# fverdoja/Fast-3D-Pointcloud-Segmentation

Hardware: AMD Instinct MI355X
Metric: Mpoints/sec segmented end-to-end, 1M-pt RGB-D frames (higher is better)
Workload: dtype f32

## Files before the change

__graft_entry__.py:

```python
import importlib
import os
import subprocess
import sys

ROOT = os.path.dirname(os.path.abspath(__file__))
PKG = "fast-3d-pointcloud-segmentation_amd"


def _run(cmd):
    print("+", " ".join(cmd), flush=True)
    subprocess.run(cmd, check=True)


def build() -> None:
    _run(["make", "-C", os.path.join(ROOT, PKG, "csrc")])
    _run(["make", "-C", os.path.join(ROOT, "oracle")])
    _run(["make", "-C", os.path.join(ROOT, "tests", "emul")])
    _run(["make", "-C", os.path.join(ROOT, "tests", "devprobe")])
    _run(["make", "-C", os.path.join(ROOT, "tests", "kernprobe")])
    _run(["make", "-C", os.path.join(ROOT, "tests", "blockprobe")])
    if ROOT not in sys.path:
        sys.path.insert(0, ROOT)
    P = importlib.import_module(PKG)
    lib = P.load_library()
    assert lib.f3ds_version() >= 120
    P.check_library_is_current(lib)


def smoke() -> None:
    import ctypes
    import numpy as np
    if ROOT not in sys.path:
        sys.path.insert(0, ROOT)
    sys.path.insert(0, os.path.join(ROOT, "tests"))
    P = importlib.import_module(PKG)
# ... 22 lines not shown
```

fast-3d-pointcloud-segmentation_amd/csrc/f3ds_hip.hip:

```cpp
#include <hip/hip_runtime.h>

#include <algorithm>
#include <cmath>
#include <atomic>
#include <map>
#include <chrono>
#include <cstdio>
#include <cstdlib>
#include <cstring>
#include <string>
#include <type_traits>
#include <mutex>
#include <set>
#include <vector>

#include "../../include/f3ds.h"
#include "f3ds_algo.h"
#include "f3ds_glasbey.h"
#include "f3ds_eval.h"
#include "f3ds_dev.h"
#include "f3ds_levels.h"
#include "f3ds_eval_levels.h"

using namespace f3ds;
// ... 45 lines not shown
template <class K>
hipError_t launch_fn(uint32_t gx, uint32_t nf, uint32_t lds, hipStream_t st, const void* dargs) {
    using Pack = pack_of<K>;
    if (lds > 48u * 1024u) {
        hipError_t e = hipFuncSetAttribute(reinterpret_cast<const void*>(k_batched<K, Pack>), hipFuncAttributeMaxDynamicSharedMemorySize, (int)lds);
        if (e != hipSuccess) return e;
    }
    hipLaunchKernelGGL((k_batched<K, Pack>), dim3(gx ? gx : 1u, nf), dim3(K::BLOCK), lds, st, static_cast<const Pack*>(dargs));
    return hipGetLastError();
}
struct Cmd { LaunchFn fn; uint32_t gx, lds, bytes, off; };

const int g_inc_shift = [] { const char* e = dev_getenv("F3DS_INC_SHIFT"); return e ? atoi(e) : 6; }();

struct Switches {
    bool direct_labels = false, copy_stream = true, copy_duplex = false, split_voxel_accum = false, sweep_tiles = true, merge_spec = true, force_global_merge = false, no_stream_pool = false, sort_pairs = false, host_prof = false, trace_err = false, vox_hash = true, vox_tiles_forced = false, levels_global = false;
    int normals_threads = 0, merge_nw = 0, merge_keys = -1; uint32_t tile_holes = 0, ilist_slack = 32, r_rounds = F3DS_R_ROUNDS, grid_cap = 0; long relabel_lds_cap = -1;
    void read() {
        auto on = [](const char* n) { return dev_getenv(n) != nullptr; };
        auto num = [](const char* n, long dflt) { const char* e = dev_getenv(n); return e ? atol(e) : dflt; };
        direct_labels = num("F3DS_DIRECT_LABELS", 0) != 0; copy_stream = num("F3DS_COPY_STREAM", 1) != 0; copy_duplex = num("F3DS_COPY_STREAM", 1) == 2; split_voxel_accum = on("F3DS_SPLIT_VOXEL_ACCUM"); sweep_tiles = num("F3DS_SWEEP_TILES", 1) != 0; merge_spec = num("F3DS_MERGE_SPEC", 1) != 0;
        force_global_merge = on("F3DS_FORCE_GLOBAL_MERGE"); no_stream_pool = on("F3DS_NO_STREAM_POOL"); sort_pairs = on("F3DS_SORT_PAIRS");
        host_prof = on("F3DS_HOST_PROF"); trace_err = on("F3DS_TRACE_ERR");
        vox_tiles_forced = num("F3DS_VOX_TILES", 1) == 2;
        vox_hash = num("F3DS_VOX_TILES", 1) != 0 && !sort_pairs && !split_voxel_accum;
        normals_threads = (int)num("F3DS_NORMALS_THREADS", 0); tile_holes = (uint32_t)num("F3DS_SWEEP_TILE_HOLES", 0);
        { const long v = num("F3DS_MERGE_NW", 0); merge_nw = v == 4 ? 4 : (v ? 8 : 0); }
        { const char* e = dev_getenv("F3DS_MERGE_KEYS"); merge_keys = !e ? -1 : (!strcmp(e, "lds") ? 2 : (!strcmp(e, "global") ? 1 : 0)); }
        relabel_lds_cap = num("F3DS_RELABEL_LDS_CAP", -1);
        levels_global = num("F3DS_LEVELS_GLOBAL", 0) != 0;
        { const long v = num("F3DS_R_ROUNDS_RUN", F3DS_R_ROUNDS); r_rounds = v >= 1 && v <= F3DS_R_ROUNDS ? (uint32_t)v : (uint32_t)F3DS_R_ROUNDS; }
        { const long v = num("F3DS_ILIST_SLACK", 32); ilist_slack = v >= 1 && v <= 32 ? (uint32_t)v : 32u; }
        { const long v = num("F3DS_GRID_CAP", 0); grid_cap = v >= 1 && v <= 2048 ? (uint32_t)v : 0u; }
    }
};
thread_local Switches g_sw;
const int g_merge_shared_res = [] { const char* e = dev_getenv("F3DS_MERGE_SHARED_RES"); return e && atoi(e) == 2 ? 2 : 0; }();

#define F3DS_SCRATCH(X) \
    X(P16, pts) X(P16, spts) X(uint64_t, keys0) X(uint64_t, keys1) X(uint32_t, vals0) X(uint32_t, vals1) X(uint32_t, flags) X(uint32_t, incl) X(uint32_t, tiles) X(uint32_t, hist) X(uint32_t, seg_start) X(int, pt_voxel) X(uint32_t, labels) \
// ... 283 lines not shown
    HIPCHECK(timed_sync(b.st));
    HIPCHECK(hipGetLastError());
    if (nf > 1) for (size_t i = 0; i < nf; ++i) *b.fr[i]->h_dc = b.owner->h_dcblk[i];
    return F3DS_OK;
}

int scan_u32(f3ds_ctx* c, const uint32_t* in, uint32_t* out, uint32_t n) {
    const uint32_t nt = n ? (n + SCAN_TILE - 1) / SCAN_TILE : 1u;
    uint32_t* tiles;
    ENSURE(c->tiles, nt, tiles);
    rec<d_scan_tiles>(c, nt, 0u, in, out, tiles, n);
    rec<d_scan_single>(c, 1u, 0u, tiles, nt);
    rec<d_scan_add>(c, nt, 0u, out, tiles, n);
    return F3DS_OK;
}
int radix_sort(f3ds_ctx* c, uint64_t* k0, uint32_t* v0, uint64_t* k1, uint32_t* v1, uint32_t n, int total_bits, uint64_t** keys_out, uint32_t** vals_out, int base_shift = 0, const uint32_t* n_dev = nullptr) {
    *keys_out = k0; if (vals_out) *vals_out = v0;
    if (total_bits <= 0) return F3DS_OK;
    const int passes = (total_bits + RS_MAXBITS - 1) / RS_MAXBITS;
    const int per = (total_bits + passes - 1) / passes;
    const uint32_t nb = n ? (n + RS_TILE - 1) / RS_TILE : 1u;
    uint32_t* hist;
    ENSURE(c->hist, (size_t)RS_BINS * nb, hist);
    int shift = 0;
    for (int p = 0; p < passes; ++p) {
        const int bits = (total_bits - shift) < per ? (total_bits - shift) : per;
        rec<d_radix_hist>(c, nb, 0u, k0, n, base_shift + shift, bits, hist, nb, n_dev);
        rec<d_scan_single>(c, 1u, 0u, hist, (uint32_t)((1u << bits) * nb));
        if (v0) rec<d_radix_scatter>(c, nb, 0u, k0, v0, k1, v1, n, base_shift + shift, bits, hist, nb, n_dev);
        else rec<d_radix_scatter_k>(c, nb, 0u, k0, k1, n, base_shift + shift, bits, hist, nb);
        std::swap(k0, k1); std::swap(v0, v1);
        shift += bits;
    }
    *keys_out = k0; if (vals_out) *vals_out = v0;
    return F3DS_OK;
}

int seg_bbox(f3ds_ctx* c) {
    rec<d_init_counters>(c, 1u, 0u, c->d_dc);
    rec<d_bbox>(c, grid_for(c->n, 256 * 8) < 512 ? grid_for(c->n, 256 * 8) : 512u, 0u, c->d_pts, c->n, c->fa, c->d_dc);
    rec<d_grid>(c, 1u, 0u, c->d_dc, c->prm.voxel_res, c->d_grid);
    return F3DS_OK;
}
int seg_sort(f3ds_ctx* c, int sort_bits, int idxbits) {
// ... 15 lines not shown
        if ((rc = scan_u32(c, flags, incl, n))) return rc;
        rec<d_segstart>(c, grid_for(n, 256), 0u, c->ks, flags, incl, n, invalid, seg_start, &c->d_dc->n_voxels, &c->d_dc->n_valid, ks);
        return F3DS_OK;
    }
    const uint32_t nt = n ? (n + SCAN_TILE - 1) / SCAN_TILE : 1u;
    uint32_t* tiles; ENSURE(c->tiles, nt, tiles);
    rec<d_seg_count>(c, nt, 0u, c->ks, n, invalid, ks, tiles);
    rec<d_scan_single>(c, 1u, 0u, tiles, nt);
    rec<d_seg_write>(c, nt, 0u, c->ks, n, invalid, ks, tiles, seg_start, &c->d_dc->n_voxels, &c->d_dc->n_valid);
    return F3DS_OK;
}
int seg_vox_tiles(f3ds_ctx* c, int code_bits, int tile_bits) {
    const uint32_t n = c->n;
    const uint32_t ntiles = (n + VT_TILE - 1u) / VT_TILE;
    const uint64_t dcap64 = (uint64_t)ntiles * VT_ENT_MAX;
    if (code_bits + tile_bits + VT_CNT_BITS > 64 || dcap64 > 0x7fffffffull || (uint64_t)ntiles * VT_TAB > 0x7fffffffull) return F3DS_ERR_UNSUPPORTED;
    const uint32_t dcap = (uint32_t)dcap64;
    const uint64_t fin = c->h_dc->n_finite;
    const uint32_t capV = (uint32_t)std::max<uint64_t>(256u, std::min<uint64_t>(fin, dcap));
    c->vox_cap = capV;
    uint64_t *k0, *k1; uint32_t *ploc, *v0, *v1, *part, *vkey, *vcount, *seg_start, *list; uint2* bo_te; float* vf; int* pt_voxel;
    const uint32_t nchunks = (dcap + DS_CHUNK - 1u) / DS_CHUNK;
    ENSURE(c->pslot, n, ploc); ENSURE(c->keys0, dcap, k0); ENSURE(c->keys1, dcap, k1); ENSURE(c->vals0, dcap, v0); ENSURE(c->vals1, dcap, v1);
    { uint32_t* w; ENSURE(c->hcnt, (size_t)ntiles * VT_TAB * 2 + 2u * nchunks, w); bo_te = reinterpret_cast<uint2*>(w); part = w + (size_t)ntiles * VT_TAB * 2; }
    ENSURE(c->vkey, (size_t)capV * 3, vkey); ENSURE(c->vcount, capV, vcount); ENSURE(c->vf, (size_t)capV * 12, vf);
    ENSURE(c->seg_start, (size_t)capV + 1, seg_start); ENSURE(c->vlist, n, list); ENSURE(c->pt_voxel, n, pt_voxel);
    { uint32_t *f, *incl; ENSURE(c->flags, capV, f); ENSURE(c->incl, capV, incl); }
    c->idxbits = -1; c->ks = nullptr; c->vs = nullptr;
    rec<d_tile_keys>(c, std::min<uint32_t>(ntiles, (uint32_t)g_grid_cap * 16u), 0u, c->d_pts, n, c->fa, c->d_grid, ploc, k0, v0, dcap, tile_bits, c->d_dc);
    uint64_t* ks; uint32_t* vs;
    int rc = radix_sort(c, k0, v0, k1, v1, dcap, code_bits + tile_bits, &ks, &vs, VT_CNT_BITS, &c->d_dc->seg_count);
    if (rc) return rc;
    rec<d_desc_part>(c, nchunks, 0u, ks, dcap, tile_bits, part, c->d_dc);
    rec<d_desc_offsets>(c, 1u, 0u, part, dcap, capV, seg_start, c->d_dc);
    rec<d_desc_apply>(c, nchunks, 0u, ks, vs, dcap, capV, tile_bits, c->fa, c->d_grid, part, bo_te, seg_start, vkey, c->d_dc);
    rec<d_tile_place>(c, std::min<uint32_t>(ntiles, (uint32_t)g_grid_cap * 16u), 0u, ploc, n, bo_te, list, pt_voxel, c->d_dc);
    rec<d_voxel_list_accum>(c, std::min<uint32_t>(grid_wide(capV, 256), std::max<uint32_t>(64u, grid_wide(n / 8u, 256))), 0u, c->d_pts, list, seg_start, c->fa, vf, vcount, c->d_dc, capV);
    c->vox_hashed = true;
    return F3DS_OK;
}
int seg_neighbors(f3ds_ctx* c, uint32_t wgs) {
    const uint32_t V = c->V;
    const bool blocks = c->h_dc->depth <= N_BLOCK_DEPTH_MAX;
    const uint32_t cap = blocks ? pow2_ge((size_t)V + 16) : pow2_ge((size_t)V * 2 + 16);
    const size_t words = blocks ? (size_t)cap * 2 : cap;
    uint32_t* hvals = nullptr; int *nbr, *nbrT; uint64_t* hkeys;
    c->hmask = cap - 1;
    ENSURE(c->nbr, (size_t)V * 27, nbr); ENSURE(c->nbrT, (size_t)V * 27, nbrT); ENSURE(c->hkeys, words, hkeys);
    if (!blocks) ENSURE(c->hvals, cap, hvals);
    rec_fill(c, hkeys, 0xFFFFFFFFu, words * 8);
    rec<d_vox_table>(c, wgs, 0u, c->vkey.p, V, c->d_grid, hkeys, hvals, c->hmask);
// ... 559 lines not shown
    bool hashed = g_sw.vox_hash && (nctx >= 4 || g_sw.vox_tiles_forced);
    for (f3ds_ctx* c : b.fr) {
        c->vox_hashed = false;
        if (c->vox_dense && hashed) { if (c->vox_dense_wait) c->vox_dense_wait--; else c->vox_dense = false; }
    }
    for (f3ds_ctx* c : b.fr) if (c->vox_dense) hashed = false;
    if (hashed) {
        uint32_t maxtiles = 1;
        for (f3ds_ctx* c : b.fr) maxtiles = std::max(maxtiles, (c->n + VT_TILE - 1u) / VT_TILE);
        const int tile_bits = bits_for((uint64_t)maxtiles - 1u);
        rc = for_frames(b, [&](f3ds_ctx* c) { return seg_vox_tiles(c, 3 * maxd, tile_bits); });
        if (rc == F3DS_ERR_UNSUPPORTED) {
            for (f3ds_ctx* c : b.fr) { reset_recording(c); c->vox_hashed = false; }
            hashed = false;
        } else if (rc || (rc = flush_sync(b))) return rc;
        if (hashed && g_sw.trace_err) for (f3ds_ctx* c : b.fr) fprintf(stderr, "f3ds: tile path: most voxels in a tile %u, descriptors %u, leaves %u, lists sorted %u\n", c->h_dc->vox_max_tile, c->h_dc->seg_count, c->h_dc->n_voxels, c->h_dc->vox_disorder);
        if (hashed) for (f3ds_ctx* c : b.fr) if (c->h_dc->ev_overflow == 6 || c->h_dc->ev_overflow == 7) {
            if (g_sw.trace_err) fprintf(stderr, "f3ds: tile path refused a frame: %s (descriptors %u, leaves %u)\n", c->h_dc->ev_overflow == 6 ? "a voxel with too many points" : "a tile with too many voxels", c->h_dc->seg_count, c->h_dc->n_voxels);
            c->vox_dense = true; c->vox_dense_wait = c->vox_dense_penalty; c->vox_dense_penalty = std::min(2u * c->vox_dense_penalty, 1024u); hashed = false;
        }
        if (!hashed) {
            if (g_sw.trace_err) fprintf(stderr, "f3ds: voxelisation of %zu frames runs again on the sort path (an unorganised cloud or dense voxels)\n", b.fr.size());
            for (f3ds_ctx* c : b.fr) {
                c->vox_hashed = false;
                if ((rc = clear_counters(c, b.st, &DevCounters::error, &DevCounters::ev_overflow, &DevCounters::n_voxels, &DevCounters::seg_count))) return rc;
            }
        }
    }
    if (!hashed) {
        uint32_t maxn = 1;
        for (f3ds_ctx* c : b.fr) if (c->n > maxn) maxn = c->n;
// ... 944 lines not shown
```

fast-3d-pointcloud-segmentation_amd/csrc/f3ds_kernels.inc:

```


namespace {

struct P16 { float x, y, z; uint32_t rgba; };

struct DevCounters {
    unsigned long long n_finite;
    uint32_t bbox[6];
    uint32_t bbox_any;
    uint32_t n_valid;
    uint32_t n_voxels;
    uint32_t n_cells;
    uint32_t n_seeds;
    uint32_t n_edges;
    uint32_t n_alive;
    uint32_t n_merges;
    uint32_t n_regions;
    uint32_t n_events;
    int error;
    int r_overflow;
    float lambda;
    uint32_t seg_count;
    uint32_t n_ghosts;
    int depth;
// ... 251 lines not shown
            uint64_t peers = __ballot(valid);
            for (int b = 0; b < bits; ++b) {
                uint64_t m = __ballot(valid && ((d >> b) & 1u));
                peers &= ((d >> b) & 1u) ? m : ~m;
            }
            uint32_t pos = 0;
            if (valid) pos = wcount[w][d] + (uint32_t)__popcll(peers & lanemask_lt());
            __builtin_amdgcn_wave_barrier();
            if (valid && (peers & lanemask_lt()) == 0ull) wcount[w][d] += (uint32_t)__popcll(peers);
            __builtin_amdgcn_wave_barrier();
            if (valid) keys_out[pos] = k[s];
        }
    }
};

struct FrameArgs {
    int use_transform, fold_negative_z, leaf_order;
    float voxel_res, seed_res, w_color, w_spatial, w_normal;
};

__device__ inline P16 load_point(const P16* pts, size_t i) {
    const uint4 q = reinterpret_cast<const uint4*>(pts)[i];
    P16 p;
    p.x = __uint_as_float(q.x); p.y = __uint_as_float(q.y); p.z = __uint_as_float(q.z); p.rgba = q.w;
    return p;
}

__device__ inline bool vt_blocks(int depth) { return depth <= N_BLOCK_DEPTH_MAX; }
constexpr uint32_t BT_EMPTY = 0xFFFFFFFFu;
struct __attribute__((aligned(16))) BtEntry { uint32_t key, base; unsigned long long vacant; };
// ... 283 lines not shown
            vcount[v] = cnt;
            uint64_t code = keys[s] >> keyshift;
            if (fa.leaf_order == 1) code = (~code) & ((1ull << (3 * depth)) - 1ull);
            unsigned k[3];
            n_demorton(code, depth, k);
            vkey[v * 3] = k[0]; vkey[v * 3 + 1] = k[1]; vkey[v * 3 + 2] = k[2];
        }
    }
};

#ifndef F3DS_VT_TILE
#define F3DS_VT_TILE 4096
#endif
constexpr uint32_t VT_TILE = F3DS_VT_TILE;
constexpr uint32_t VT_TAB = VT_TILE / 2;
constexpr int VT_CNT_BITS = 14;
static_assert(VT_TILE < (1u << VT_CNT_BITS), "a tile's point count must fit the count field");
constexpr uint32_t VT_ENT_MAX = VT_TAB * 5 / 8;
constexpr uint32_t VL_MAX_RUN = 256;
constexpr uint32_t VOX_NONE = 0xFFFFFFFFu;
__device__ inline void run_of_lane(bool valid, uint32_t w0, uint32_t w1, bool* head, int* head_lane, uint32_t* run_len) {
    const int lane = lane_id();
    const uint32_t p0 = __shfl_up(w0, 1, 64), p1 = __shfl_up(w1, 1, 64);
    const bool pv = __shfl_up((int)valid, 1, 64) != 0;
    const bool h = valid && (lane == 0 || !pv || p0 != w0 || p1 != w1);
    const uint64_t hm = __ballot(h), vm = __ballot(valid);
    const uint64_t le = lane == 63 ? ~0ull : ((2ull << lane) - 1ull);
    const int hl = valid ? 63 - __builtin_clzll(hm & le) : lane;
    const uint64_t above = hl == 63 ? 0ull : ~((2ull << hl) - 1ull);
    const uint64_t stop = (hm | ~vm) & above;
    *head = h; *head_lane = hl; *run_len = (uint32_t)((stop ? __builtin_ctzll(stop) : 64) - hl);
}
struct d_tile_keys {
    static constexpr int BLOCK = 256;
    __device__ void operator()(const P16* pts, uint32_t n, FrameArgs fa, const GridInfo* gp, uint32_t* ploc, uint64_t* dkeys, uint32_t* dvals,
                               uint32_t dcap, int tile_bits, DevCounters* dc) const {
        __shared__ unsigned long long tkey[VT_TAB];
        __shared__ uint32_t tcnt[VT_TAB];
        __shared__ uint32_t tbits[2][VT_TAB / 32];
        __shared__ uint32_t s_ent, s_base, s_over[2], s_dis;
        const GridInfo g = *gp;
        const uint64_t code_mask = (1ull << (3 * g.depth)) - 1ull;
        const int lane = lane_id();
        const uint32_t tid = threadIdx.x;
        const uint32_t ntiles = (n + VT_TILE - 1u) / VT_TILE;
        for (uint32_t tile = BIX; tile < ntiles; tile += gridDim.x) {
            for (uint32_t e = tid; e < VT_TAB; e += 256u) { tkey[e] = HASH_EMPTY; tcnt[e] = 0u; }
            if (tid < VT_TAB / 32u) { tbits[0][tid] = 0u; tbits[1][tid] = 0u; }
            if (tid == 0) { s_ent = 0u; s_over[0] = 0u; s_over[1] = 0u; s_dis = 0u; }
            __syncthreads();
            const uint32_t t0 = tile * VT_TILE, t1 = n - t0 < VT_TILE ? n : t0 + VT_TILE;
            constexpr uint32_t VT_PF = 4;
            uint32_t it4 = 0u;
            for (uint32_t base4 = t0; base4 < t1 && !s_over[(it4 + 1u) & 1u]; base4 += 256u * VT_PF, ++it4) {
              uint4 q[VT_PF];
        #pragma unroll
              for (uint32_t j = 0; j < VT_PF; ++j) { const uint32_t i = base4 + j * 256u + tid; q[j] = reinterpret_cast<const uint4*>(pts)[i < t1 ? i : t1 - 1u]; }
        #pragma unroll
              for (uint32_t j = 0; j < VT_PF; ++j) {
                const uint32_t base = base4 + j * 256u;
                if (base >= t1) break;
                const uint32_t i = base + tid;
                const uint32_t step = (base - t0) >> 8;
                uint64_t pk = HASH_EMPTY;
                if (i < t1) {
                    float x = __uint_as_float(q[j].x), y = __uint_as_float(q[j].y), z = __uint_as_float(q[j].z);
                    n_prelude(z, fa.fold_negative_z);
                    if (n_finite3(x, y, z) && !g.empty) { unsigned k[3]; n_point_key(g, x, y, z, fa.use_transform, k); pk = n_pack_key(k[0], k[1], k[2]); }
                }
// ... 5 lines not shown
                    uint32_t e = (uint32_t)hash64(pk) & (VT_TAB - 1u);
                    for (uint32_t probes = 0; probes < VT_TAB; ++probes) {
                        const unsigned long long old = atomicCAS(&tkey[e], (unsigned long long)HASH_EMPTY, (unsigned long long)pk);
                        if (old == HASH_EMPTY) { if (atomicAdd(&s_ent, 1u) >= VT_ENT_MAX) s_over[it4 & 1u] = 1u; ent = e; break; }
                        if (old == pk) { ent = e; break; }
                        e = (e + 1u) & (VT_TAB - 1u);
                    }
                    if (ent != VOX_NONE) {
                        roff = atomicAdd(&tcnt[ent], len);
                        const uint32_t bit = 1u << (ent & 31u);
                        if (atomicOr(&tbits[step & 1u][ent >> 5], bit) & bit) s_dis = 1u;
                    } else s_over[it4 & 1u] = 1u;
                }
                if (tid < VT_TAB / 32u) tbits[(step + 1u) & 1u][tid] = 0u;
                ent = __shfl(ent, hl, 64); roff = __shfl(roff, hl, 64);
                if (i < t1) ploc[i] = (valid && ent != VOX_NONE) ? (ent << 16) | (roff + (uint32_t)(lane - hl)) : VOX_NONE;
                __syncthreads();
              }
            }
            __syncthreads();
            if (tid == 0) { atomicMax(&dc->vox_max_tile, s_ent); if (s_dis) dc->vox_disorder = 1u; }
            if (s_over[0] | s_over[1]) { if (tid == 0) { dc->error = F3DS_ERR_UNSUPPORTED; dc->ev_overflow = 7; } return; }
            if (tid == 0) s_base = s_ent ? atomicAdd(&dc->seg_count, s_ent) : 0u;
            __syncthreads();
            const uint32_t dbase = s_base;
            if (tid == 0) s_ent = 0u;
            __syncthreads();
            for (uint32_t e0 = 0; e0 < VT_TAB; e0 += 256u) {
                const uint32_t e = e0 + tid;
                const unsigned long long pk = tkey[e];
                const bool live = pk != HASH_EMPTY;
                const uint64_t lm = __ballot(live);
                if (!lm) continue;
                uint32_t wb = 0;
                if (lane == __builtin_ctzll(lm)) wb = atomicAdd(&s_ent, (uint32_t)__popcll(lm));
                wb = __shfl(wb, __builtin_ctzll(lm), 64);
                if (live) {
                    const uint32_t d = dbase + wb + (uint32_t)__popcll(lm & lanemask_lt());
                    if (d < dcap) {
                        uint64_t code = n_morton((unsigned)(pk >> 42) & 0x1FFFFFu, (unsigned)(pk >> 21) & 0x1FFFFFu, (unsigned)pk & 0x1FFFFFu, g.depth);
                        if (fa.leaf_order == 1) code = (~code) & code_mask;
                        dkeys[d] = (((code << tile_bits) | (uint64_t)tile) << VT_CNT_BITS) | (uint64_t)tcnt[e];
                        dvals[d] = tile * VT_TAB + e;
                    } else { dc->error = F3DS_ERR_UNSUPPORTED; dc->ev_overflow = 7; }
                }
            }
            __syncthreads();
        }
    }
};
constexpr uint32_t DS_IT = 8;
constexpr uint32_t DS_CHUNK = 256u * DS_IT;
struct DescThread { uint64_t code[DS_IT]; uint32_t te[DS_IT], cnt[DS_IT]; uint32_t headmask, nheads, npts; };
__device__ inline void desc_load(const uint64_t* dkeys, const uint32_t* dvals, uint32_t D, int tile_bits, uint32_t db, DescThread& t, bool want_te) {
    const int sh = tile_bits + VT_CNT_BITS;
    uint64_t prev = (db > 0u && db - 1u < D) ? dkeys[db - 1u] >> sh : ~0ull;
#pragma unroll
    for (uint32_t k = 0; k < DS_IT; ++k) {
        const uint32_t d = db + k;
        const uint64_t key = d < D ? dkeys[d] : 0ull;
        t.code[k] = key >> sh; t.cnt[k] = d < D ? (uint32_t)key & ((1u << VT_CNT_BITS) - 1u) : 0u;
        t.te[k] = (want_te && d < D) ? dvals[d] : 0u;
    }
    t.headmask = 0u; t.nheads = 0u; t.npts = 0u;
#pragma unroll
    for (uint32_t k = 0; k < DS_IT; ++k) {
        const uint32_t d = db + k;
        const bool head = d < D && (d == 0u || prev != t.code[k]);
        prev = t.code[k];
        if (head) { t.headmask |= 1u << k; t.nheads++; }
        t.npts += t.cnt[k];
    }
}
__device__ inline void block_excl_scan2(uint32_t a, uint32_t b, uint32_t* ea, uint32_t* eb, uint32_t* ta, uint32_t* tb) {
    __shared__ uint32_t s_a[4], s_b[4];
    const uint32_t lane = (uint32_t)lane_id(), w = threadIdx.x >> 6;
    uint32_t ia = a, ib = b;
#pragma unroll
    for (int k = 1; k < 64; k <<= 1) { const uint32_t x = __shfl_up(ia, k, 64), y = __shfl_up(ib, k, 64); if ((int)lane >= k) { ia += x; ib += y; } }
    __syncthreads();
    if (lane == 63u) { s_a[w] = ia; s_b[w] = ib; }
    __syncthreads();
    uint32_t ba = 0, bb = 0, sa = 0, sb = 0;
#pragma unroll
    for (uint32_t k = 0; k < 4u; ++k) { if (k < w) { ba += s_a[k]; bb += s_b[k]; } sa += s_a[k]; sb += s_b[k]; }
    *ea = ba + ia - a; *eb = bb + ib - b; *ta = sa; *tb = sb;
}
struct d_desc_part {
    static constexpr int BLOCK = 256;
    __device__ void operator()(const uint64_t* dkeys, uint32_t dcap, int tile_bits, uint32_t* part, const DevCounters* dc) const {
        if (dc->ev_overflow) return;
        const uint32_t D = dc->seg_count < dcap ? dc->seg_count : dcap;
        const uint32_t nchunks = (dcap + DS_CHUNK - 1u) / DS_CHUNK;
        for (uint32_t b = BIX; b < nchunks; b += gridDim.x) {
            DescThread t;
            desc_load(dkeys, nullptr, D, tile_bits, b * DS_CHUNK + threadIdx.x * DS_IT, t, false);
            uint32_t eh, ec, th, tc;
            block_excl_scan2(t.nheads, t.npts, &eh, &ec, &th, &tc);
            if (threadIdx.x == 0) { part[2u * b] = th; part[2u * b + 1u] = tc; }
            __syncthreads();
        }
    }
};
struct d_desc_offsets {
    static constexpr bool LATENCY_KERNEL = true;
    static constexpr int BLOCK = 256;
    __device__ void operator()(uint32_t* part, uint32_t dcap, uint32_t capV, uint32_t* seg_start, DevCounters* dc) const {
        if (BIX || dc->ev_overflow) return;
        const uint32_t nchunks = (dcap + DS_CHUNK - 1u) / DS_CHUNK;
        uint32_t ch = 0, cc = 0;
        for (uint32_t b0 = 0; b0 < nchunks; b0 += 256u) {
// ... 1 lines not shown
            const uint32_t h = b < nchunks ? part[2u * b] : 0u, c = b < nchunks ? part[2u * b + 1u] : 0u;
            uint32_t eh, ec, th, tc;
            block_excl_scan2(h, c, &eh, &ec, &th, &tc);
            if (b < nchunks) { part[2u * b] = ch + eh; part[2u * b + 1u] = cc + ec; }
            ch += th; cc += tc;
            __syncthreads();
        }
        if (threadIdx.x == 0) {
            dc->n_voxels = ch; dc->n_valid = cc;
            if (ch <= capV) seg_start[ch] = cc; else { dc->error = F3DS_ERR_UNSUPPORTED; dc->ev_overflow = 7; }
        }
    }
};
struct d_desc_apply {
    static constexpr int BLOCK = 256;
    __device__ void operator()(const uint64_t* dkeys, const uint32_t* dvals, uint32_t dcap, uint32_t capV, int tile_bits, FrameArgs fa, const GridInfo* gp,
                               const uint32_t* part, uint2* bo_te, uint32_t* seg_start, uint32_t* vkey, const DevCounters* dc) const {
        if (dc->ev_overflow) return;
        const uint32_t D = dc->seg_count < dcap ? dc->seg_count : dcap;
        const int depth = gp->depth;
        const uint32_t nchunks = (D + DS_CHUNK - 1u) / DS_CHUNK;
        for (uint32_t b = BIX; b < nchunks; b += gridDim.x) {
            const uint32_t db = b * DS_CHUNK + threadIdx.x * DS_IT;
            DescThread t;
            desc_load(dkeys, dvals, D, tile_bits, db, t, true);
            uint32_t eh, ec, th, tc;
            block_excl_scan2(t.nheads, t.npts, &eh, &ec, &th, &tc);
            uint32_t ord = part[2u * b] + eh;
            uint32_t pos = part[2u * b + 1u] + ec;
        #pragma unroll
            for (uint32_t k = 0; k < DS_IT; ++k) {
                if (db + k >= D) break;
                if (t.headmask & (1u << k)) {
                    if (ord < capV) {
                        seg_start[ord] = pos;
                        uint64_t c2 = t.code[k];
                        if (fa.leaf_order == 1) c2 = (~c2) & ((1ull << (3 * depth)) - 1ull);
                        unsigned k3[3];
                        n_demorton(c2, depth, k3);
                        vkey[ord * 3] = k3[0]; vkey[ord * 3 + 1] = k3[1]; vkey[ord * 3 + 2] = k3[2];
                    }
                    ord++;
                }
                bo_te[t.te[k]] = make_uint2(pos, ord - 1u);
                pos += t.cnt[k];
            }
            __syncthreads();
        }
    }
};
struct d_tile_place {
    static constexpr int BLOCK = 256;
    __device__ void operator()(const uint32_t* ploc, uint32_t n, const uint2* bo_te, uint32_t* list, int* pt_voxel, const DevCounters* dc) const {
        __shared__ uint2 tab[VT_TAB];
        if (dc->ev_overflow) return;
        const uint32_t ntiles = (n + VT_TILE - 1u) / VT_TILE;
        for (uint32_t tile = BIX; tile < ntiles; tile += gridDim.x) {
            const uint32_t t0 = tile * VT_TILE, t1 = n - t0 < VT_TILE ? n : t0 + VT_TILE;
            constexpr uint32_t PF = 4;
            uint32_t pl[PF];
    #pragma unroll
            for (uint32_t j = 0; j < PF; ++j) { const uint32_t i = t0 + j * 256u + threadIdx.x; pl[j] = i < t1 ? ploc[i] : VOX_NONE; }
            __syncthreads();
            for (uint32_t e = threadIdx.x; e < VT_TAB; e += 256u) tab[e] = bo_te[(size_t)tile * VT_TAB + e];
            __syncthreads();
            for (uint32_t i0 = t0; i0 < t1; i0 += 256u * PF) {
                uint32_t nx[PF];
    #pragma unroll
                for (uint32_t j = 0; j < PF; ++j) { const uint32_t i = i0 + (PF + j) * 256u + threadIdx.x; nx[j] = i < t1 ? ploc[i] : VOX_NONE; }
    #pragma unroll
                for (uint32_t j = 0; j < PF; ++j) {
                    const uint32_t i = i0 + j * 256u + threadIdx.x;
                    if (i >= t1) continue;
                    if (pl[j] == VOX_NONE) { pt_voxel[i] = -1; continue; }
                    const uint2 bo = tab[pl[j] >> 16];
                    list[bo.x + (pl[j] & 0xFFFFu)] = i;
                    pt_voxel[i] = (int)bo.y;
                }
    #pragma unroll
// ... 3206 lines not shown
```

fast-3d-pointcloud-segmentation_amd/csrc/f3ds_numerics.h:

```cpp
#ifndef F3DS_NUMERICS_H_
#define F3DS_NUMERICS_H_

#include "f3ds_math.h"

namespace f3ds {

#define F3DS_FLT_MAX 3.402823466e+38f
#define F3DS_FLT_MIN 1.175494351e-38f
#define F3DS_FLT_EPS 1.192092896e-07f

F3DS_HD float n_sqrtf(float x) { return __builtin_sqrtf(x); }
F3DS_HD double n_sqrt(double x) { return __builtin_sqrt(x); }
F3DS_HD bool n_finite3(float x, float y, float z) { return m_isfinitef(x) && m_isfinitef(y) && m_isfinitef(z); }
F3DS_HD float n_nanf() { return m_from_bitsf(0x7fc00000u); }

struct GridInfo {
    double min[3];
    double max[3];
    double res;
    int depth;
    unsigned max_key;
    int error;
    int empty;
};
// ... 81 lines not shown
        y = (y << 1) | ((d >> 1) & 1u);
        z = (z << 1) | (d & 1u);
    }
    key[0] = x; key[1] = y; key[2] = z;
}
F3DS_HD uint64_t n_pack_key(unsigned x, unsigned y, unsigned z) {
    return ((uint64_t)x << 42) | ((uint64_t)y << 21) | (uint64_t)z;
}
#define N_BLOCK_DEPTH_MAX 12
F3DS_HD uint32_t n_block_key(unsigned x, unsigned y, unsigned z) { return ((x >> 2) << 20) | ((y >> 2) << 10) | (z >> 2); }
F3DS_HD unsigned n_block_cell(unsigned x, unsigned y, unsigned z) { return (unsigned)n_morton(x & 3u, y & 3u, z & 3u, 2); }
F3DS_HD int n_block_ordinal(uint32_t base, uint64_t mask, unsigned cell, int leaf_order) {
    if (!((mask >> cell) & 1ull)) return -1;
    const uint64_t before = leaf_order == 1 ? ((mask >> cell) >> 1) : (mask & ((1ull << cell) - 1ull));
    return (int)(base + (uint32_t)__builtin_popcountll(before));
}

F3DS_HD void n_roots2(float b, float c, float r[3]) {
    r[0] = 0.0f;
    float d = (float)((double)(b * b) - 4.0 * (double)c);
    if (d < 0.0f) d = 0.0f;
    float sd = n_sqrtf(d);
    r[2] = 0.5f * (b + sd);
    r[1] = 0.5f * (b - sd);
}
template <class K = m_lit> F3DS_HD void n_roots(float m00, float m01, float m02, float m11, float m12, float m22, float r[3], K mc = K()) {
    float c0 = m00 * m11 * m22 + 2.0f * m01 * m02 * m12 - m00 * m12 * m12 - m11 * m02 * m02 - m22 * m01 * m01;
    float c1 = m00 * m11 - m01 * m01 + m00 * m22 - m02 * m02 + m11 * m22 - m12 * m12;
    float c2 = m00 + m11 + m22;
    if (m_absf(c0) < F3DS_FLT_EPS) { n_roots2(c2, c1, r); return; }
// ... 206 lines not shown
```

Measured before the change: 3719.

## Pack voxel descriptors into one sortable word with per-tile fixed slots

Voxel descriptors now sit at fixed per-tile slots (tile*VT_ENT_MAX+cid) instead of being compacted with a global atomic. When the bits fit, the tile, dense entry id and count are packed into one 64-bit key, so the separate value arrays and key-value sort go away. The radix sort only sorts the Morton code bits, skipping the tile bits. Its first pass uses new segmented histogram and scatter kernels that mask out the unused slots in each tile. Point slots are rewritten to dense ids so the placement table reads only the live entries, at the cost of a larger sparse sort input and more kernel variants.

Result: slower. 3653 (-1.8%).

```diff
diff --git a/__graft_entry__.py b/__graft_entry__.py
--- a/__graft_entry__.py
+++ b/__graft_entry__.py
@@ -19,6 +19,7 @@
     _run(["make", "-C", os.path.join(ROOT, "tests", "devprobe")])
     _run(["make", "-C", os.path.join(ROOT, "tests", "kernprobe")])
     _run(["make", "-C", os.path.join(ROOT, "tests", "blockprobe")])
+    _run(["make", "-C", os.path.join(ROOT, "tests", "descprobe")])
     if ROOT not in sys.path:
         sys.path.insert(0, ROOT)
     P = importlib.import_module(PKG)
diff --git a/fast-3d-pointcloud-segmentation_amd/csrc/f3ds_hip.hip b/fast-3d-pointcloud-segmentation_amd/csrc/f3ds_hip.hip
--- a/fast-3d-pointcloud-segmentation_amd/csrc/f3ds_hip.hip
+++ b/fast-3d-pointcloud-segmentation_amd/csrc/f3ds_hip.hip
@@ -83,7 +83,7 @@
 const int g_inc_shift = [] { const char* e = dev_getenv("F3DS_INC_SHIFT"); return e ? atoi(e) : 6; }();
 
 struct Switches {
-    bool direct_labels = false, copy_stream = true, copy_duplex = false, split_voxel_accum = false, sweep_tiles = true, merge_spec = true, force_global_merge = false, no_stream_pool = false, sort_pairs = false, host_prof = false, trace_err = false, vox_hash = true, vox_tiles_forced = false, levels_global = false;
+    bool direct_labels = false, copy_stream = true, copy_duplex = false, split_voxel_accum = false, sweep_tiles = true, merge_spec = true, force_global_merge = false, no_stream_pool = false, sort_pairs = false, host_prof = false, trace_err = false, vox_hash = true, vox_tiles_forced = false, levels_global = false, desc_pairs = false;
     int normals_threads = 0, merge_nw = 0, merge_keys = -1; uint32_t tile_holes = 0, ilist_slack = 32, r_rounds = F3DS_R_ROUNDS, grid_cap = 0; long relabel_lds_cap = -1;
     void read() {
         auto on = [](const char* n) { return dev_getenv(n) != nullptr; };
@@ -93,6 +93,7 @@
         host_prof = on("F3DS_HOST_PROF"); trace_err = on("F3DS_TRACE_ERR");
         vox_tiles_forced = num("F3DS_VOX_TILES", 1) == 2;
         vox_hash = num("F3DS_VOX_TILES", 1) != 0 && !sort_pairs && !split_voxel_accum;
+        desc_pairs = num("F3DS_DESC_PAIRS", 0) != 0;
         normals_threads = (int)num("F3DS_NORMALS_THREADS", 0); tile_holes = (uint32_t)num("F3DS_SWEEP_TILE_HOLES", 0);
         { const long v = num("F3DS_MERGE_NW", 0); merge_nw = v == 4 ? 4 : (v ? 8 : 0); }
         { const char* e = dev_getenv("F3DS_MERGE_KEYS"); merge_keys = !e ? -1 : (!strcmp(e, "lds") ? 2 : (!strcmp(e, "global") ? 1 : 0)); }
@@ -406,10 +407,13 @@
     rec<d_scan_add>(c, nt, 0u, out, tiles, n);
     return F3DS_OK;
 }
-int radix_sort(f3ds_ctx* c, uint64_t* k0, uint32_t* v0, uint64_t* k1, uint32_t* v1, uint32_t n, int total_bits, uint64_t** keys_out, uint32_t** vals_out, int base_shift = 0, const uint32_t* n_dev = nullptr) {
+int radix_sort(f3ds_ctx* c, uint64_t* k0, uint32_t* v0, uint64_t* k1, uint32_t* v1, uint32_t n, int total_bits, uint64_t** keys_out, uint32_t** vals_out, int base_shift = 0, const uint32_t* n_dev = nullptr,
+               const uint32_t* seg_cnt = nullptr, uint32_t seg_len = 0) {
     *keys_out = k0; if (vals_out) *vals_out = v0;
-    if (total_bits <= 0) return F3DS_OK;
-    const int passes = (total_bits + RS_MAXBITS - 1) / RS_MAXBITS;
+    if (seg_cnt && (!seg_len || !n_dev)) return F3DS_ERR_LOGIC;
+    if (total_bits <= 0 && !seg_cnt) return F3DS_OK;
+    if (total_bits < 0) total_bits = 0;
+    const int passes = std::max((total_bits + RS_MAXBITS - 1) / RS_MAXBITS, 1);
     const int per = (total_bits + passes - 1) / passes;
     const uint32_t nb = n ? (n + RS_TILE - 1) / RS_TILE : 1u;
     uint32_t* hist;
@@ -417,9 +421,14 @@
     int shift = 0;
     for (int p = 0; p < passes; ++p) {
         const int bits = (total_bits - shift) < per ? (total_bits - shift) : per;
-        rec<d_radix_hist>(c, nb, 0u, k0, n, base_shift + shift, bits, hist, nb, n_dev);
+        const bool seg = seg_cnt && p == 0;
+        if (seg) rec<d_radix_hist_seg>(c, nb, 0u, k0, seg_cnt, n / seg_len, seg_len, base_shift + shift, bits, hist, nb);
+        else rec<d_radix_hist>(c, nb, 0u, k0, n, base_shift + shift, bits, hist, nb, n_dev);
         rec<d_scan_single>(c, 1u, 0u, hist, (uint32_t)((1u << bits) * nb));
-        if (v0) rec<d_radix_scatter>(c, nb, 0u, k0, v0, k1, v1, n, base_shift + shift, bits, hist, nb, n_dev);
+        if (seg && v0) rec<d_radix_scatter_seg>(c, nb, 0u, k0, v0, k1, v1, seg_cnt, n / seg_len, seg_len, base_shift + shift, bits, hist, nb);
+        else if (seg) rec<d_radix_scatter_seg_k>(c, nb, 0u, k0, k1, seg_cnt, n / seg_len, seg_len, base_shift + shift, bits, hist, nb);
+        else if (v0) rec<d_radix_scatter>(c, nb, 0u, k0, v0, k1, v1, n, base_shift + shift, bits, hist, nb, n_dev);
+        else if (n_dev) rec<d_radix_scatter_kn>(c, nb, 0u, k0, k1, n, base_shift + shift, bits, hist, nb, n_dev);
         else rec<d_radix_scatter_k>(c, nb, 0u, k0, k1, n, base_shift + shift, bits, hist, nb);
         std::swap(k0, k1); std::swap(v0, v1);
         shift += bits;
@@ -465,27 +474,30 @@
     const uint32_t n = c->n;
     const uint32_t ntiles = (n + VT_TILE - 1u) / VT_TILE;
     const uint64_t dcap64 = (uint64_t)ntiles * VT_ENT_MAX;
-    if (code_bits + tile_bits + VT_CNT_BITS > 64 || dcap64 > 0x7fffffffull || (uint64_t)ntiles * VT_TAB > 0x7fffffffull) return F3DS_ERR_UNSUPPORTED;
+    const int one_word = n_desc_one_word(code_bits, tile_bits) && !g_sw.desc_pairs;
+    if ((!one_word && code_bits + VT_CNT_BITS > 64) || dcap64 > 0x7fffffffull) return F3DS_ERR_UNSUPPORTED;
+    const int code_shift = n_desc_code_shift(tile_bits, one_word);
     const uint32_t dcap = (uint32_t)dcap64;
     const uint64_t fin = c->h_dc->n_finite;
     const uint32_t capV = (uint32_t)std::max<uint64_t>(256u, std::min<uint64_t>(fin, dcap));
     c->vox_cap = capV;
-    uint64_t *k0, *k1; uint32_t *ploc, *v0, *v1, *part, *vkey, *vcount, *seg_start, *list; uint2* bo_te; float* vf; int* pt_voxel;
+    uint64_t *k0, *k1; uint32_t *ploc, *v0 = nullptr, *v1 = nullptr, *part, *tcount, *vkey, *vcount, *seg_start, *list; uint2* bo_te; float* vf; int* pt_voxel;
     const uint32_t nchunks = (dcap + DS_CHUNK - 1u) / DS_CHUNK;
-    ENSURE(c->pslot, n, ploc); ENSURE(c->keys0, dcap, k0); ENSURE(c->keys1, dcap, k1); ENSURE(c->vals0, dcap, v0); ENSURE(c->vals1, dcap, v1);
-    { uint32_t* w; ENSURE(c->hcnt, (size_t)ntiles * VT_TAB * 2 + 2u * nchunks, w); bo_te = reinterpret_cast<uint2*>(w); part = w + (size_t)ntiles * VT_TAB * 2; }
+    ENSURE(c->pslot, n, ploc); ENSURE(c->keys0, dcap, k0); ENSURE(c->keys1, dcap, k1);
+    if (!one_word) { ENSURE(c->vals0, dcap, v0); ENSURE(c->vals1, dcap, v1); }
+    { uint32_t* w; ENSURE(c->hcnt, (size_t)dcap * 2 + 2u * nchunks + ntiles, w); bo_te = reinterpret_cast<uint2*>(w); part = w + (size_t)dcap * 2; tcount = part + 2u * nchunks; }
     ENSURE(c->vkey, (size_t)capV * 3, vkey); ENSURE(c->vcount, capV, vcount); ENSURE(c->vf, (size_t)capV * 12, vf);
     ENSURE(c->seg_start, (size_t)capV + 1, seg_start); ENSURE(c->vlist, n, list); ENSURE(c->pt_voxel, n, pt_voxel);
     { uint32_t *f, *incl; ENSURE(c->flags, capV, f); ENSURE(c->incl, capV, incl); }
     c->idxbits = -1; c->ks = nullptr; c->vs = nullptr;
-    rec<d_tile_keys>(c, std::min<uint32_t>(ntiles, (uint32_t)g_grid_cap * 16u), 0u, c->d_pts, n, c->fa, c->d_grid, ploc, k0, v0, dcap, tile_bits, c->d_dc);
+    rec<d_tile_keys>(c, std::min<uint32_t>(ntiles, (uint32_t)g_grid_cap * 16u), 0u, c->d_pts, n, c->fa, c->d_grid, ploc, k0, v0, tcount, tile_bits, c->d_dc);
     uint64_t* ks; uint32_t* vs;
-    int rc = radix_sort(c, k0, v0, k1, v1, dcap, code_bits + tile_bits, &ks, &vs, VT_CNT_BITS, &c->d_dc->seg_count);
+    int rc = radix_sort(c, k0, v0, k1, v1, dcap, code_bits, &ks, &vs, code_shift, &c->d_dc->seg_count, tcount, VT_ENT_MAX);
     if (rc) return rc;
-    rec<d_desc_part>(c, nchunks, 0u, ks, dcap, tile_bits, part, c->d_dc);
+    rec<d_desc_part>(c, nchunks, 0u, ks, dcap, code_shift, part, c->d_dc);
     rec<d_desc_offsets>(c, 1u, 0u, part, dcap, capV, seg_start, c->d_dc);
-    rec<d_desc_apply>(c, nchunks, 0u, ks, vs, dcap, capV, tile_bits, c->fa, c->d_grid, part, bo_te, seg_start, vkey, c->d_dc);
-    rec<d_tile_place>(c, std::min<uint32_t>(ntiles, (uint32_t)g_grid_cap * 16u), 0u, ploc, n, bo_te, list, pt_voxel, c->d_dc);
+    rec<d_desc_apply>(c, nchunks, 0u, ks, vs, dcap, capV, code_shift, tile_bits, c->fa, c->d_grid, part, bo_te, seg_start, vkey, c->d_dc);
+    rec<d_tile_place>(c, std::min<uint32_t>(ntiles, (uint32_t)g_grid_cap * 16u), 0u, ploc, n, bo_te, tcount, list, pt_voxel, c->d_dc);
     rec<d_voxel_list_accum>(c, std::min<uint32_t>(grid_wide(capV, 256), std::max<uint32_t>(64u, grid_wide(n / 8u, 256))), 0u, c->d_pts, list, seg_start, c->fa, vf, vcount, c->d_dc, capV);
     c->vox_hashed = true;
     return F3DS_OK;
@@ -1075,7 +1087,8 @@
             for (f3ds_ctx* c : b.fr) { reset_recording(c); c->vox_hashed = false; }
             hashed = false;
         } else if (rc || (rc = flush_sync(b))) return rc;
-        if (hashed && g_sw.trace_err) for (f3ds_ctx* c : b.fr) fprintf(stderr, "f3ds: tile path: most voxels in a tile %u, descriptors %u, leaves %u, lists sorted %u\n", c->h_dc->vox_max_tile, c->h_dc->seg_count, c->h_dc->n_voxels, c->h_dc->vox_disorder);
+        if (hashed && g_sw.trace_err) for (f3ds_ctx* c : b.fr) fprintf(stderr, "f3ds: tile path: most voxels in a tile %u, descriptors %u (%s, sorted on %d code bits), leaves %u, lists sorted %u\n", c->h_dc->vox_max_tile, c->h_dc->seg_count,
+                                                                       n_desc_one_word(3 * maxd, tile_bits) && !g_sw.desc_pairs ? "one word each" : "pairs", 3 * maxd, c->h_dc->n_voxels, c->h_dc->vox_disorder);
         if (hashed) for (f3ds_ctx* c : b.fr) if (c->h_dc->ev_overflow == 6 || c->h_dc->ev_overflow == 7) {
             if (g_sw.trace_err) fprintf(stderr, "f3ds: tile path refused a frame: %s (descriptors %u, leaves %u)\n", c->h_dc->ev_overflow == 6 ? "a voxel with too many points" : "a tile with too many voxels", c->h_dc->seg_count, c->h_dc->n_voxels);
             c->vox_dense = true; c->vox_dense_wait = c->vox_dense_penalty; c->vox_dense_penalty = std::min(2u * c->vox_dense_penalty, 1024u); hashed = false;
diff --git a/fast-3d-pointcloud-segmentation_amd/csrc/f3ds_kernels.inc b/fast-3d-pointcloud-segmentation_amd/csrc/f3ds_kernels.inc
--- a/fast-3d-pointcloud-segmentation_amd/csrc/f3ds_kernels.inc
+++ b/fast-3d-pointcloud-segmentation_amd/csrc/f3ds_kernels.inc
@@ -289,6 +289,110 @@
     }
 };
 
+template <bool PAIRS>
+__device__ __forceinline__ void rs_scatter_masked(const uint64_t* keys, const uint32_t* vals, uint64_t* keys_out, uint32_t* vals_out, int shift, int bits,
+                                                  const uint32_t* hist_scanned, uint32_t nblocks, uint32_t vm) {
+    __shared__ uint32_t wcount[RS_WAVES][RS_BINS];
+    const uint32_t mask = (1u << bits) - 1u;
+    const int w = threadIdx.x >> 6;
+    for (int i = threadIdx.x; i < RS_WAVES * RS_BINS; i += RS_THREADS) (&wcount[0][0])[i] = 0;
+    __syncthreads();
+    const uint32_t wbase = BIX * RS_TILE + w * (64 * RS_STRIPS);
+    uint64_t k[RS_STRIPS];
+#pragma unroll
+    for (int s = 0; s < RS_STRIPS; ++s) {
+        const uint32_t i = wbase + s * 64 + lane_id();
+        const bool valid = (vm >> s) & 1u;
+        k[s] = valid ? keys[i] : 0ull;
+        if (valid) atomicAdd(&wcount[w][(uint32_t)(k[s] >> shift) & mask], 1u);
+    }
+    __syncthreads();
+    for (uint32_t d = threadIdx.x; d < (1u << bits); d += RS_THREADS) {
+        uint32_t run = hist_scanned[d * nblocks + BIX];
+        for (int ww = 0; ww < RS_WAVES; ++ww) { uint32_t t = wcount[ww][d]; wcount[ww][d] = run; run += t; }
+    }
+    __syncthreads();
+#pragma unroll
+    for (int s = 0; s < RS_STRIPS; ++s) {
+        const uint32_t i = wbase + s * 64 + lane_id();
+        const bool valid = (vm >> s) & 1u;
+        uint64_t peers = __ballot(valid);
+        if (!peers) continue;
+        const uint32_t d = (uint32_t)(k[s] >> shift) & mask;
+        for (int b = 0; b < bits; ++b) {
+            uint64_t m = __ballot(valid && ((d >> b) & 1u));
+            peers &= ((d >> b) & 1u) ? m : ~m;
+        }
+        uint32_t pos = 0;
+        if (valid) pos = wcount[w][d] + (uint32_t)__popcll(peers & lanemask_lt());
+        __builtin_amdgcn_wave_barrier();
+        if (valid && (peers & lanemask_lt()) == 0ull) wcount[w][d] += (uint32_t)__popcll(peers);
+        __builtin_amdgcn_wave_barrier();
+        if (valid) { keys_out[pos] = k[s]; if (PAIRS) vals_out[pos] = vals[i]; }
+    }
+}
+__device__ inline uint32_t rs_valid_below(uint32_t n) {
+    const uint32_t wbase = BIX * RS_TILE + (threadIdx.x >> 6) * (64 * RS_STRIPS);
+    uint32_t vm = 0u;
+#pragma unroll
+    for (int s = 0; s < RS_STRIPS; ++s) if (wbase + s * 64 + lane_id() < n) vm |= 1u << s;
+    return vm;
+}
+__device__ inline uint32_t rs_valid_seg(const uint32_t* seg_cnt, uint32_t nsegs, uint32_t seg_len) {
+    const uint32_t i0 = BIX * RS_TILE + (threadIdx.x >> 6) * (64 * RS_STRIPS) + lane_id();
+    uint32_t t = i0 / seg_len, r = i0 % seg_len, vm = 0u;
+#pragma unroll
+    for (int s = 0; s < RS_STRIPS; ++s) {
+        if (t < nsegs && r < seg_cnt[t]) vm |= 1u << s;
+        r += 64u;
+        while (r >= seg_len) { r -= seg_len; ++t; }
+    }
+    return vm;
+}
+struct d_radix_scatter_kn {
+    static constexpr int BLOCK = RS_THREADS;
+    __device__ void operator()(const uint64_t* keys, uint64_t* keys_out, uint32_t n, int shift, int bits, const uint32_t* hist_scanned, uint32_t nblocks, const uint32_t* n_dev) const {
+        if (BIX >= nblocks) return;
+        if (n_dev) { const uint32_t nd = *n_dev; n = nd < n ? nd : n; }
+        rs_scatter_masked<false>(keys, nullptr, keys_out, nullptr, shift, bits, hist_scanned, nblocks, rs_valid_below(n));
+    }
+};
+struct d_radix_hist_seg {
+    static constexpr int BLOCK = RS_THREADS;
+    __device__ void operator()(const uint64_t* keys, const uint32_t* seg_cnt, uint32_t nsegs, uint32_t seg_len, int shift, int bits, uint32_t* hist, uint32_t nblocks) const {
+        if (BIX >= nblocks) return;
+        __shared__ uint32_t lh[RS_BINS];
+        for (int i = threadIdx.x; i < RS_BINS; i += RS_THREADS) lh[i] = 0;
+        __syncthreads();
+        const uint32_t mask = (1u << bits) - 1u;
+        const uint32_t wbase = BIX * RS_TILE + (threadIdx.x >> 6) * (64 * RS_STRIPS);
+        const uint32_t vm = rs_valid_seg(seg_cnt, nsegs, seg_len);
+    #pragma unroll
+        for (int s = 0; s < RS_STRIPS; ++s) {
+            const uint32_t i = wbase + s * 64 + lane_id();
+            if ((vm >> s) & 1u) atomicAdd(&lh[(uint32_t)(keys[i] >> shift) & mask], 1u);
+        }
+        __syncthreads();
+        for (uint32_t d = threadIdx.x; d < (1u << bits); d += RS_THREADS) hist[d * nblocks + BIX] = lh[d];
+    }
+};
+struct d_radix_scatter_seg {
+    static constexpr int BLOCK = RS_THREADS;
+    __device__ void operator()(const uint64_t* keys, const uint32_t* vals, uint64_t* keys_out, uint32_t* vals_out, const uint32_t* seg_cnt, uint32_t nsegs, uint32_t seg_len,
+                               int shift, int bits, const uint32_t* hist_scanned, uint32_t nblocks) const {
+        if (BIX >= nblocks) return;
+        rs_scatter_masked<true>(keys, vals, keys_out, vals_out, shift, bits, hist_scanned, nblocks, rs_valid_seg(seg_cnt, nsegs, seg_len));
+    }
+};
+struct d_radix_scatter_seg_k {
+    static constexpr int BLOCK = RS_THREADS;
+    __device__ void operator()(const uint64_t* keys, uint64_t* keys_out, const uint32_t* seg_cnt, uint32_t nsegs, uint32_t seg_len, int shift, int bits,
+                               const uint32_t* hist_scanned, uint32_t nblocks) const {
+        if (BIX >= nblocks) return;
+        rs_scatter_masked<false>(keys, nullptr, keys_out, nullptr, shift, bits, hist_scanned, nblocks, rs_valid_seg(seg_cnt, nsegs, seg_len));
+    }
+};
+
 struct FrameArgs {
     int use_transform, fold_negative_z, leaf_order;
     float voxel_res, seed_res, w_color, w_spatial, w_normal;
@@ -602,9 +706,11 @@
 #endif
 constexpr uint32_t VT_TILE = F3DS_VT_TILE;
 constexpr uint32_t VT_TAB = VT_TILE / 2;
-constexpr int VT_CNT_BITS = 14;
+constexpr int VT_CNT_BITS = N_DESC_CNT_BITS;
 static_assert(VT_TILE < (1u << VT_CNT_BITS), "a tile's point count must fit the count field");
 constexpr uint32_t VT_ENT_MAX = VT_TAB * 5 / 8;
+static_assert(VT_ENT_MAX <= (1u << N_DESC_CID_BITS), "a tile's dense entry ids must fit their field of the descriptor (and the upper half of a per-point word)");
+constexpr uint32_t VT_STEPS = VT_TILE / 256u;
 constexpr uint32_t VL_MAX_RUN = 256;
 constexpr uint32_t VOX_NONE = 0xFFFFFFFFu;
 __device__ inline void run_of_lane(bool valid, uint32_t w0, uint32_t w1, bool* head, int* head_lane, uint32_t* run_len) {
@@ -622,11 +728,12 @@
 struct d_tile_keys {
     static constexpr int BLOCK = 256;
     __device__ void operator()(const P16* pts, uint32_t n, FrameArgs fa, const GridInfo* gp, uint32_t* ploc, uint64_t* dkeys, uint32_t* dvals,
-                               uint32_t dcap, int tile_bits, DevCounters* dc) const {
+                               uint32_t* tcount, int tile_bits, DevCounters* dc) const {
         __shared__ unsigned long long tkey[VT_TAB];
         __shared__ uint32_t tcnt[VT_TAB];
+        __shared__ uint16_t tcid[VT_TAB];
         __shared__ uint32_t tbits[2][VT_TAB / 32];
-        __shared__ uint32_t s_ent, s_base, s_over[2], s_dis;
+        __shared__ uint32_t s_ent, s_over[2], s_dis;
         const GridInfo g = *gp;
         const uint64_t code_mask = (1ull << (3 * g.depth)) - 1ull;
         const int lane = lane_id();
@@ -639,8 +746,14 @@
             __syncthreads();
             const uint32_t t0 = tile * VT_TILE, t1 = n - t0 < VT_TILE ? n : t0 + VT_TILE;
             constexpr uint32_t VT_PF = 4;
-            uint32_t it4 = 0u;
-            for (uint32_t base4 = t0; base4 < t1 && !s_over[(it4 + 1u) & 1u]; base4 += 256u * VT_PF, ++it4) {
+            static_assert(VT_STEPS % VT_PF == 0, "whole rounds of VT_PF steps");
+            uint32_t pw[VT_STEPS];
+        #pragma unroll
+            for (uint32_t k = 0; k < VT_STEPS; ++k) pw[k] = VOX_NONE;
+        #pragma unroll
+            for (uint32_t it4 = 0u; it4 < VT_STEPS / VT_PF; ++it4) {
+              const uint32_t base4 = t0 + it4 * 256u * VT_PF;
+              if (base4 >= t1 || s_over[(it4 + 1u) & 1u]) break;
               uint4 q[VT_PF];
         #pragma unroll
               for (uint32_t j = 0; j < VT_PF; ++j) { const uint32_t i = base4 + j * 256u + tid; q[j] = reinterpret_cast<const uint4*>(pts)[i < t1 ? i : t1 - 1u]; }
@@ -676,17 +789,14 @@
                 }
                 if (tid < VT_TAB / 32u) tbits[(step + 1u) & 1u][tid] = 0u;
                 ent = __shfl(ent, hl, 64); roff = __shfl(roff, hl, 64);
-                if (i < t1) ploc[i] = (valid && ent != VOX_NONE) ? (ent << 16) | (roff + (uint32_t)(lane - hl)) : VOX_NONE;
+                if (i < t1 && valid && ent != VOX_NONE) pw[it4 * VT_PF + j] = (ent << 16) | (roff + (uint32_t)(lane - hl));
                 __syncthreads();
               }
             }
             __syncthreads();
             if (tid == 0) { atomicMax(&dc->vox_max_tile, s_ent); if (s_dis) dc->vox_disorder = 1u; }
             if (s_over[0] | s_over[1]) { if (tid == 0) { dc->error = F3DS_ERR_UNSUPPORTED; dc->ev_overflow = 7; } return; }
-            if (tid == 0) s_base = s_ent ? atomicAdd(&dc->seg_count, s_ent) : 0u;
-            __syncthreads();
-            const uint32_t dbase = s_base;
-            if (tid == 0) s_ent = 0u;
+            if (tid == 0) { tcount[tile] = s_ent; if (s_ent) atomicAdd(&dc->seg_count, s_ent); s_ent = 0u; }
             __syncthreads();
             for (uint32_t e0 = 0; e0 < VT_TAB; e0 += 256u) {
                 const uint32_t e = e0 + tid;
@@ -698,14 +808,22 @@
                 if (lane == __builtin_ctzll(lm)) wb = atomicAdd(&s_ent, (uint32_t)__popcll(lm));
                 wb = __shfl(wb, __builtin_ctzll(lm), 64);
                 if (live) {
-                    const uint32_t d = dbase + wb + (uint32_t)__popcll(lm & lanemask_lt());
-                    if (d < dcap) {
+                    const uint32_t cid = wb + (uint32_t)__popcll(lm & lanemask_lt());
+                    tcid[e] = (uint16_t)cid;
+                    if (cid < VT_ENT_MAX) {
+                        const uint32_t d = tile * VT_ENT_MAX + cid;
                         uint64_t code = n_morton((unsigned)(pk >> 42) & 0x1FFFFFu, (unsigned)(pk >> 21) & 0x1FFFFFu, (unsigned)pk & 0x1FFFFFu, g.depth);
                         if (fa.leaf_order == 1) code = (~code) & code_mask;
-                        dkeys[d] = (((code << tile_bits) | (uint64_t)tile) << VT_CNT_BITS) | (uint64_t)tcnt[e];
-                        dvals[d] = tile * VT_TAB + e;
-                    } else { dc->error = F3DS_ERR_UNSUPPORTED; dc->ev_overflow = 7; }
-                }
+                        dkeys[d] = n_desc_key(code, tile, cid, tcnt[e], tile_bits, dvals == nullptr);
+                        if (dvals) dvals[d] = d;
+                    }
+                }
+            }
+            __syncthreads();
+        #pragma unroll
+            for (uint32_t k = 0; k < VT_STEPS; ++k) {
+                const uint32_t i = t0 + k * 256u + tid;
+                if (i < t1) ploc[i] = pw[k] == VOX_NONE ? VOX_NONE : ((uint32_t)tcid[pw[k] >> 16] << 16) | (pw[k] & 0xFFFFu);
             }
             __syncthreads();
         }
@@ -714,15 +832,14 @@
 constexpr uint32_t DS_IT = 8;
 constexpr uint32_t DS_CHUNK = 256u * DS_IT;
 struct DescThread { uint64_t code[DS_IT]; uint32_t te[DS_IT], cnt[DS_IT]; uint32_t headmask, nheads, npts; };
-__device__ inline void desc_load(const uint64_t* dkeys, const uint32_t* dvals, uint32_t D, int tile_bits, uint32_t db, DescThread& t, bool want_te) {
-    const int sh = tile_bits + VT_CNT_BITS;
+__device__ inline void desc_load(const uint64_t* dkeys, const uint32_t* dvals, uint32_t D, int sh, int tile_bits, uint32_t db, DescThread& t, bool want_te) {
     uint64_t prev = (db > 0u && db - 1u < D) ? dkeys[db - 1u] >> sh : ~0ull;
 #pragma unroll
     for (uint32_t k = 0; k < DS_IT; ++k) {
         const uint32_t d = db + k;
         const uint64_t key = d < D ? dkeys[d] : 0ull;
-        t.code[k] = key >> sh; t.cnt[k] = d < D ? (uint32_t)key & ((1u << VT_CNT_BITS) - 1u) : 0u;
-        t.te[k] = (want_te && d < D) ? dvals[d] : 0u;
+        t.code[k] = key >> sh; t.cnt[k] = d < D ? n_desc_count(key) : 0u;
+        t.te[k] = (want_te && d < D) ? (dvals ? dvals[d] : n_desc_slot(key, tile_bits, VT_ENT_MAX)) : 0u;
     }
     t.headmask = 0u; t.nheads = 0u; t.npts = 0u;
 #pragma unroll
@@ -750,13 +867,13 @@
 }
 struct d_desc_part {
     static constexpr int BLOCK = 256;
-    __device__ void operator()(const uint64_t* dkeys, uint32_t dcap, int tile_bits, uint32_t* part, const DevCounters* dc) const {
+    __device__ void operator()(const uint64_t* dkeys, uint32_t dcap, int code_shift, uint32_t* part, const DevCounters* dc) const {
         if (dc->ev_overflow) return;
         const uint32_t D = dc->seg_count < dcap ? dc->seg_count : dcap;
         const uint32_t nchunks = (dcap + DS_CHUNK - 1u) / DS_CHUNK;
         for (uint32_t b = BIX; b < nchunks; b += gridDim.x) {
             DescThread t;
-            desc_load(dkeys, nullptr, D, tile_bits, b * DS_CHUNK + threadIdx.x * DS_IT, t, false);
+            desc_load(dkeys, nullptr, D, code_shift, 0, b * DS_CHUNK + threadIdx.x * DS_IT, t, false);
             uint32_t eh, ec, th, tc;
             block_excl_scan2(t.nheads, t.npts, &eh, &ec, &th, &tc);
             if (threadIdx.x == 0) { part[2u * b] = th; part[2u * b + 1u] = tc; }
@@ -788,7 +905,7 @@
 };
 struct d_desc_apply {
     static constexpr int BLOCK = 256;
-    __device__ void operator()(const uint64_t* dkeys, const uint32_t* dvals, uint32_t dcap, uint32_t capV, int tile_bits, FrameArgs fa, const GridInfo* gp,
+    __device__ void operator()(const uint64_t* dkeys, const uint32_t* dvals, uint32_t dcap, uint32_t capV, int code_shift, int tile_bits, FrameArgs fa, const GridInfo* gp,
                                const uint32_t* part, uint2* bo_te, uint32_t* seg_start, uint32_t* vkey, const DevCounters* dc) const {
         if (dc->ev_overflow) return;
         const uint32_t D = dc->seg_count < dcap ? dc->seg_count : dcap;
@@ -797,7 +914,7 @@
         for (uint32_t b = BIX; b < nchunks; b += gridDim.x) {
             const uint32_t db = b * DS_CHUNK + threadIdx.x * DS_IT;
             DescThread t;
-            desc_load(dkeys, dvals, D, tile_bits, db, t, true);
+            desc_load(dkeys, dvals, D, code_shift, tile_bits, db, t, true);
             uint32_t eh, ec, th, tc;
             block_excl_scan2(t.nheads, t.npts, &eh, &ec, &th, &tc);
             uint32_t ord = part[2u * b] + eh;
@@ -816,7 +933,7 @@
                     }
                     ord++;
                 }
-                bo_te[t.te[k]] = make_uint2(pos, ord - 1u);
+                if (t.te[k] < dcap) bo_te[t.te[k]] = make_uint2(pos, ord - 1u);
                 pos += t.cnt[k];
             }
             __syncthreads();
@@ -825,8 +942,8 @@
 };
 struct d_tile_place {
     static constexpr int BLOCK = 256;
-    __device__ void operator()(const uint32_t* ploc, uint32_t n, const uint2* bo_te, uint32_t* list, int* pt_voxel, const DevCounters* dc) const {
-        __shared__ uint2 tab[VT_TAB];
+    __device__ void operator()(const uint32_t* ploc, uint32_t n, const uint2* bo_te, const uint32_t* tcount, uint32_t* list, int* pt_voxel, const DevCounters* dc) const {
+        __shared__ uint2 tab[VT_ENT_MAX];
         if (dc->ev_overflow) return;
         const uint32_t ntiles = (n + VT_TILE - 1u) / VT_TILE;
         for (uint32_t tile = BIX; tile < ntiles; tile += gridDim.x) {
@@ -836,7 +953,8 @@
     #pragma unroll
             for (uint32_t j = 0; j < PF; ++j) { const uint32_t i = t0 + j * 256u + threadIdx.x; pl[j] = i < t1 ? ploc[i] : VOX_NONE; }
             __syncthreads();
-            for (uint32_t e = threadIdx.x; e < VT_TAB; e += 256u) tab[e] = bo_te[(size_t)tile * VT_TAB + e];
+            const uint32_t live = tcount[tile] < VT_ENT_MAX ? tcount[tile] : VT_ENT_MAX;
+            for (uint32_t e = threadIdx.x; e < live; e += 256u) tab[e] = bo_te[(size_t)tile * VT_ENT_MAX + e];
             __syncthreads();
             for (uint32_t i0 = t0; i0 < t1; i0 += 256u * PF) {
                 uint32_t nx[PF];
diff --git a/fast-3d-pointcloud-segmentation_amd/csrc/f3ds_numerics.h b/fast-3d-pointcloud-segmentation_amd/csrc/f3ds_numerics.h
--- a/fast-3d-pointcloud-segmentation_amd/csrc/f3ds_numerics.h
+++ b/fast-3d-pointcloud-segmentation_amd/csrc/f3ds_numerics.h
@@ -119,6 +119,19 @@
     if (!((mask >> cell) & 1ull)) return -1;
     const uint64_t before = leaf_order == 1 ? ((mask >> cell) >> 1) : (mask & ((1ull << cell) - 1ull));
     return (int)(base + (uint32_t)__builtin_popcountll(before));
+}
+#define N_DESC_CNT_BITS 14
+#define N_DESC_CID_BITS 11
+F3DS_HD int n_desc_one_word(int code_bits, int tile_bits) { return code_bits + tile_bits + N_DESC_CID_BITS + N_DESC_CNT_BITS <= 64; }
+F3DS_HD int n_desc_code_shift(int tile_bits, int one_word) { return one_word ? tile_bits + N_DESC_CID_BITS + N_DESC_CNT_BITS : N_DESC_CNT_BITS; }
+F3DS_HD uint64_t n_desc_key(uint64_t code, uint32_t tile, uint32_t cid, uint32_t count, int tile_bits, int one_word) {
+    if (!one_word) return (code << N_DESC_CNT_BITS) | (uint64_t)count;
+    return (((((code << tile_bits) | (uint64_t)tile) << N_DESC_CID_BITS) | (uint64_t)cid) << N_DESC_CNT_BITS) | (uint64_t)count;
+}
+F3DS_HD uint32_t n_desc_count(uint64_t key) { return (uint32_t)key & ((1u << N_DESC_CNT_BITS) - 1u); }
+F3DS_HD uint32_t n_desc_slot(uint64_t key, int tile_bits, uint32_t ent_stride) {
+    const uint64_t tc = (key >> N_DESC_CNT_BITS) & ((1ull << (tile_bits + N_DESC_CID_BITS)) - 1ull);
+    return (uint32_t)(tc >> N_DESC_CID_BITS) * ent_stride + ((uint32_t)tc & ((1u << N_DESC_CID_BITS) - 1u));
 }
 
 F3DS_HD void n_roots2(float b, float c, float r[3]) {
```
